# yuke93/ReconfigISP

Hardware: AMD Instinct MI355X
Metric: MPix/s end-to-end 5-stage ISP forward, 256x256 Bayer (higher is better)
Workload: dtype f32; 1 GPU; batch=64 256x256 Bayer per GPU, 5-stage fixed ISP forward Demosaic_01_sRGB_07_11_01_14 (nearest demosaic, bilateral denoise, WbManual, Gamma, GtmManual; OriginUniversal), all stage outputs materialised; global_batch=64, parallelism=batch-sharded x1, no collective

## Files before the change

reconfigisp_amd/csrc/risp_fused.hip:

```cpp
#include "risp_common.h"
#include "risp_ops.h"

namespace {

using namespace risp_ops;

constexpr int FX = 64, FY = 16, PXT = 4;

struct FusedArgs {
    const float *in;
    float *out_dem;
    float *out_bil;
    const int *win;
    const float *sig_c, *sig_s;
    int n_ops, N, H, W, R;
    int last_out;
    int ops[RISP_MAX_CHAIN];
    const float *params[RISP_MAX_CHAIN];
    float *outs[RISP_MAX_CHAIN];
};

__device__ __forceinline__ int refl(int i, int n) {
    if (i < 0) i = -i;
    if (i >= n) i = 2 * n - 2 - i;
    return i < 0 ? 0 : (i >= n ? n - 1 : i);
}
typedef float v4f __attribute__((ext_vector_type(4)));
__device__ __forceinline__ void st4_nt(float *p, v4f v) {
#ifndef RISP_STREAM_POLICY
#define RISP_STREAM_POLICY "nt"
#endif
    asm volatile("global_store_dwordx4 %0, %1, off " RISP_STREAM_POLICY ::"v"(p), "v"(v) : "memory");
}
__device__ __forceinline__ float q8f(float v) {
    return floorf(__builtin_amdgcn_fmed3f(v, 0.f, 255.f) + 0.5f);
}

template <bool FROM_BAYER, int RT, bool WBQ>
#ifndef RISP_FUSED_WAVES
#define RISP_FUSED_WAVES 1
#endif
__global__ __launch_bounds__(256, RISP_FUSED_WAVES) void bilateral_chain_kernel(const FusedArgs a) {
    extern __shared__ float lds[];
    const int R = RT > 0 ? RT : a.R, H = a.H, W = a.W;
    const int tw = FX + 2 * R, th = FY + 2 * R, per = tw * th;
#ifndef RISP_FUSED_NO_XCD_MAP
    int bxi = blockIdx.x, byi = blockIdx.y, bzi = blockIdx.z;
    {
        const unsigned total = gridDim.x * gridDim.y * gridDim.z;
        if ((total & 7u) == 0) {
            const unsigned lin = blockIdx.x + gridDim.x * (blockIdx.y + gridDim.y * blockIdx.z);
            const unsigned t = (lin & 7u) * (total >> 3) + (lin >> 3);
            bxi = t % gridDim.x;
            byi = (t / gridDim.x) % gridDim.y;
            bzi = t / (gridDim.x * gridDim.y);
        }
    }
    const int n = bzi, x0 = bxi * FX, y0 = byi * FY;
#else
    const int n = blockIdx.z, x0 = blockIdx.x * FX, y0 = blockIdx.y * FY;
#endif
    const size_t plane = (size_t)H * W;

    const int lx = (threadIdx.x & 15) * PXT, ly = threadIdx.x >> 4;
    const int px = x0 + lx, py = y0 + ly;
    if (FROM_BAYER && RT == 1) {
        constexpr int TWc = FX + 2, THc = FY + 2, PERc = TWc * THc, QW = FX / 2 + 2, QH = FY / 2 + 2;
        const float *bay = a.in + (size_t)n * plane;
        float2 top[2], bot[2];
#pragma unroll
        for (int it = 0; it < 2; ++it) {
            const int q = threadIdx.x + 256 * it;
            const int j = q / QW, i = q - j * QW;
            const int Y = y0 - 2 + 2 * j, X = x0 - 2 + 2 * i;
            const bool ok = q < QW * QH && Y >= 0 && Y < H && X >= 0 && X < W;
            top[it] = ok ? *reinterpret_cast<const float2 *>(bay + (size_t)Y * W + X) : make_float2(0.f, 0.f);
            bot[it] = ok ? *reinterpret_cast<const float2 *>(bay + (size_t)(Y + 1) * W + X) : make_float2(0.f, 0.f);
        }
#pragma unroll
        for (int it = 0; it < 2; ++it) {
            const int q = threadIdx.x + 256 * it;
            const int j = q / QW, i = q - j * QW;
            const int Y = y0 - 2 + 2 * j, X = x0 - 2 + 2 * i;
            if (!(q < QW * QH && Y >= 0 && Y < H && X >= 0 && X < W)) continue;
            const float R_ = top[it].x, G1 = top[it].y, G2 = bot[it].x, B_ = bot[it].y;
#pragma unroll
            for (int dy = 0; dy < 2; ++dy)
#pragma unroll
                for (int dx = 0; dx < 2; ++dx) {
                    const int ty = 2 * j - 1 + dy, tx = 2 * i - 1 + dx;
                    if (ty >= 0 && ty < THc && tx >= 0 && tx < TWc) {
                        const int idx = ty * TWc + tx;
                        lds[idx] = B_;
                        lds[PERc + idx] = dy ? G2 : G1;
                        lds[2 * PERc + idx] = R_;
                    }
                }
        }
        if (x0 == 0 || y0 == 0 || x0 + FX >= W || y0 + FY >= H) {
            __syncthreads();
            for (int idx = threadIdx.x; idx < PERc; idx += 256) {
                const int ty = idx / TWc, tx = idx - ty * TWc;
                const int gy = y0 - 1 + ty, gx = x0 - 1 + tx;
                if (gy >= 0 && gy < H && gx >= 0 && gx < W) continue;
                const int sy = refl(gy, H) - (y0 - 1), sx = refl(gx, W) - (x0 - 1);
                if (sy < 0 || sy >= THc || sx < 0 || sx >= TWc) continue;
                const int src = sy * TWc + sx;
                lds[idx] = lds[src];
                lds[PERc + idx] = lds[PERc + src];
                lds[2 * PERc + idx] = lds[2 * PERc + src];
            }
        }
    } else if (FROM_BAYER) {
        const float *bay = a.in + (size_t)n * plane;
        for (int idx = threadIdx.x; idx < per; idx += 256) {
            const int ty = idx / tw, tx = idx - ty * tw;
            const int gy = refl(y0 + ty - R, H), gx = refl(x0 + tx - R, W);
            const int qy = gy & ~1, qx = gx & ~1;
            lds[2 * per + idx] = bay[(size_t)qy * W + qx];
            lds[per + idx] = bay[(size_t)(qy + (gy & 1)) * W + qx + 1 - (gy & 1)];
            lds[idx] = bay[(size_t)(qy + 1) * W + qx + 1];
        }
    } else {
        const float *img = a.in + (size_t)n * 3 * plane;
        auto fetch1 = [&](int idx) {
            const int c = idx / per, rem = idx - c * per;
            const int ty = rem / tw, tx = rem - ty * tw;
            return img[(size_t)c * plane + (size_t)refl(y0 + ty - R, H) * W + refl(x0 + tx - R, W)];
        };
        if (RT > 0) {
            constexpr int PER3 = 3 * (FX + 2 * RT) * (FY + 2 * RT), NIT = (PER3 + 255) / 256;
            float v[NIT];
#pragma unroll
            for (int i = 0; i < NIT; ++i) {
                const int idx = threadIdx.x + 256 * i;
                v[i] = idx < PER3 ? fetch1(idx) : 0.f;
            }
#pragma unroll
            for (int i = 0; i < NIT; ++i) {
                const int idx = threadIdx.x + 256 * i;
                if (idx < PER3) lds[idx] = v[i];
            }
        } else {
            for (int idx = threadIdx.x; idx < 3 * per; idx += 256) lds[idx] = fetch1(idx);
        }
    }
    __syncthreads();

    if (px >= W || py >= H) return;
    const size_t o = (size_t)n * 3 * plane + (size_t)py * W + px;
    const float *ctr = lds + (ly + R) * tw + lx + R;

    if (FROM_BAYER) {
        float4 vb, vg, vr;
        float *eb = reinterpret_cast<float *>(&vb), *eg = reinterpret_cast<float *>(&vg), *er = reinterpret_cast<float *>(&vr);
#pragma unroll
        for (int i = 0; i < PXT; ++i) {
            eb[i] = ctr[i];
            eg[i] = ctr[per + i];
            er[i] = ctr[2 * per + i];
        }
        st4_nt(a.out_dem + o, *reinterpret_cast<v4f *>(&vb));
        st4_nt(a.out_dem + o + plane, *reinterpret_cast<v4f *>(&vg));
        st4_nt(a.out_dem + o + 2 * plane, *reinterpret_cast<v4f *>(&vr));
    }

    int r = a.win[n] / 2;
    r = r < 0 ? 0 : (r > R ? R : r);
    const bool full = RT > 0 && r == RT;
    const float ks = -1.f / (2.f * a.sig_s[n] * a.sig_s[n]), kc = -1.f / (2.f * a.sig_c[n] * a.sig_c[n]);
    const float ks2 = ks * 1.4426950408889634f, kc2 = kc * 1.4426950408889634f;
    f3 pix[PXT];
#pragma unroll
    for (int i = 0; i < PXT; ++i) {
        const float *c0 = ctr + i;
        const float cb = c0[0] * 255.f, cg = c0[per] * 255.f, cr = c0[2 * per] * 255.f;
        float nb = 0.f, ng = 0.f, nr = 0.f, den = 0.f;
        auto tap = [&](int dy, int dx) {
            if (dy == 0 && dx == 0) {
                nb += cb; ng += cg; nr += cr; den += 1.f;
                return;
            }
            const float *q = c0 + dy * tw + dx;
            const float qb = q[0] * 255.f, qg = q[per] * 255.f, qr = q[2 * per] * 255.f;
            const float dist = fabsf(qb - cb) + fabsf(qg - cg) + fabsf(qr - cr);
            const float wgt = __builtin_amdgcn_exp2f(__builtin_fmaf(dist * dist, kc2, (float)(dy * dy + dx * dx) * ks2));
            nb = __builtin_fmaf(wgt, qb, nb); ng = __builtin_fmaf(wgt, qg, ng); nr = __builtin_fmaf(wgt, qr, nr); den += wgt;
        };
        if (full) {
#pragma unroll
            for (int dy = -RT; dy <= RT; ++dy)
#pragma unroll
                for (int dx = -RT; dx <= RT; ++dx) tap(dy, dx);
        } else {
            for (int dy = -r; dy <= r; ++dy)
                for (int dx = -r; dx <= r; ++dx) tap(dy, dx);
        }
        const float inv255 = 1.f / 255.f, rden = 1.f / den;
        pix[i] = {q8f(nb * rden) * inv255, q8f(ng * rden) * inv255, q8f(nr * rden) * inv255};
    }
    auto store = [&](float *dst, bool stream) {
        const v4f vb = {pix[0].b, pix[1].b, pix[2].b, pix[3].b}, vg = {pix[0].g, pix[1].g, pix[2].g, pix[3].g},
                  vr = {pix[0].r, pix[1].r, pix[2].r, pix[3].r};
        if (stream) {
            st4_nt(dst + o, vb);
            st4_nt(dst + o + plane, vg);
            st4_nt(dst + o + 2 * plane, vr);
        } else {
            *reinterpret_cast<v4f *>(dst + o) = vb;
            *reinterpret_cast<v4f *>(dst + o + plane) = vg;
            *reinterpret_cast<v4f *>(dst + o + 2 * plane) = vr;
        }
    };
    store(a.out_bil, a.last_out >= 0);

    for (int k = 0; k < a.n_ops; ++k) {
        apply_op<PXT, WBQ>(a.ops[k], a.params[k], n, pix);
        if (a.outs[k]) store(a.outs[k], k < a.last_out);
    }
}

}

extern "C" {

int risp_bilateral_chain_fwd(const float *in, int from_bayer, float *out_demosaic, float *out_bilateral,
                             const int32_t *window, const float *sigma_color, const float *sigma_space, int max_window,
                             int n_ops, const int *ops, const float *const *params, float *const *outs, int N, int H,
                             int W, void *stream) {
    RISP_CHECK_ARG(in && out_bilateral && window && sigma_color && sigma_space, "risp_bilateral_chain_fwd: null argument");
    RISP_CHECK_ARG(!from_bayer || out_demosaic, "risp_bilateral_chain_fwd: demosaic output buffer missing");
    RISP_CHECK_ARG(n_ops >= 0 && n_ops <= RISP_MAX_CHAIN && (n_ops == 0 || (ops && params && outs)),
                   "risp_bilateral_chain_fwd: bad op list");
    RISP_CHECK_ARG(max_window >= 1 && max_window <= 17 && (max_window & 1), "risp_bilateral_chain_fwd: window %d", max_window);
    RISP_CHECK_ARG(N > 0 && N <= 65535 && H % 2 == 0 && W % 4 == 0 && H > max_window / 2 && W > max_window / 2,
                   "risp_bilateral_chain_fwd: bad shape N=%d H=%d W=%d (W must be a multiple of 4)", N, H, W);
    FusedArgs a;
    a.in = in;
    a.out_dem = out_demosaic;
    a.out_bil = out_bilateral;
    a.win = window;
    a.sig_c = sigma_color;
    a.sig_s = sigma_space;
    a.n_ops = n_ops;
    a.N = N;
    a.H = H;
    a.W = W;
    a.R = max_window / 2;
    a.last_out = -1;
    for (int k = 0; k < RISP_MAX_CHAIN; ++k) {
        a.ops[k] = RISP_OP_SKIP;
        a.params[k] = nullptr;
        a.outs[k] = nullptr;
    }
    for (int k = 0; k < n_ops; ++k) {
        RISP_CHECK_ARG(ops[k] == RISP_OP_SKIP || (ops[k] >= RISP_OP_WB_MANUAL && ops[k] <= RISP_OP_GAIN3),
                       "risp_bilateral_chain_fwd: op %d not allowed after the stencil", ops[k]);
        RISP_CHECK_ARG(ops[k] == RISP_OP_SKIP || (params[k] && outs[k]), "risp_bilateral_chain_fwd: stage %d incomplete", k);
        a.ops[k] = ops[k];
        a.params[k] = params[k];
        a.outs[k] = ops[k] == RISP_OP_SKIP ? nullptr : outs[k];
        if (a.outs[k]) a.last_out = k;
    }
#ifdef RISP_NT_ALL
    a.last_out = RISP_MAX_CHAIN;
#endif
    const size_t lds = sizeof(float) * 3 * (FX + 2 * a.R) * (FY + 2 * a.R);
    dim3 grid((W + FX - 1) / FX, (H + FY - 1) / FY, N);
    hipStream_t s = (hipStream_t)stream;
    bool wbq = false;
    for (int k = 0; k < n_ops; ++k) wbq |= a.ops[k] == RISP_OP_WB_QUADRATIC;
#ifdef RISP_CHAIN_ALWAYS_WBQ
    wbq = true;
#endif
#define RISP_FUSED_LAUNCH(FB, RTV)                                                                            \
    do {                                                                                                      \
        if (wbq) hipLaunchKernelGGL((bilateral_chain_kernel<FB, RTV, true>), grid, dim3(256), lds, s, a);     \
        else hipLaunchKernelGGL((bilateral_chain_kernel<FB, RTV, false>), grid, dim3(256), lds, s, a);        \
    } while (0)
    if (a.R == 1) {
        if (from_bayer) RISP_FUSED_LAUNCH(true, 1);
        else RISP_FUSED_LAUNCH(false, 1);
    } else {
        if (from_bayer) RISP_FUSED_LAUNCH(true, 0);
        else RISP_FUSED_LAUNCH(false, 0);
    }
#undef RISP_FUSED_LAUNCH
    RISP_LAUNCH_CHECK("risp_bilateral_chain_fwd");
    return 0;
}

const char *risp_bilateral_chain_kernel(int from_bayer, int max_window, int with_wb_quadratic) {
    static const char *names[2][2][2] = {
        {{"bilateral_chain_kernel<false,0,false>", "bilateral_chain_kernel<false,0,true>"},
         {"bilateral_chain_kernel<false,1,false>", "bilateral_chain_kernel<false,1,true>"}},
        {{"bilateral_chain_kernel<true,0,false>", "bilateral_chain_kernel<true,0,true>"},
         {"bilateral_chain_kernel<true,1,false>", "bilateral_chain_kernel<true,1,true>"}}};
    return names[from_bayer ? 1 : 0][max_window / 2 == 1 ? 1 : 0][with_wb_quadratic ? 1 : 0];
}

}
```

Before: 89660 MPix/s.

## Add register-only quad kernel for Bayer demosaic plus 3x3 bilateral chain

Adds a new kernel for the Bayer-input, radius-1 case. Each thread loads a 6x8 Bayer neighbourhood straight from global memory into registers, does the nearest demosaic and 3x3 bilateral filter on a 2x4 output patch, then runs the rest of the op chain, with no LDS and no barriers. The aim is to drop the shared-memory staging, the syncs and the tile halo overhead, in exchange for redundant global loads across neighbouring threads and more register pressure. The XCD remap is also moved into a helper, and the inline-asm nontemporal store gains an s_nop, while the new path uses the builtin nontemporal store.

```diff
diff --git a/reconfigisp_amd/csrc/risp_fused.hip b/reconfigisp_amd/csrc/risp_fused.hip
--- a/reconfigisp_amd/csrc/risp_fused.hip
+++ b/reconfigisp_amd/csrc/risp_fused.hip
@@ -30,10 +30,28 @@
 #ifndef RISP_STREAM_POLICY
 #define RISP_STREAM_POLICY "nt"
 #endif
-    asm volatile("global_store_dwordx4 %0, %1, off " RISP_STREAM_POLICY ::"v"(p), "v"(v) : "memory");
+    asm volatile("global_store_dwordx4 %0, %1, off " RISP_STREAM_POLICY "\n\ts_nop 1" ::"v"(p), "v"(v) : "memory");
+}
+__device__ __forceinline__ void st4_stream(float *p, v4f v) {
+    asm("" : "+v"(v));
+    __builtin_nontemporal_store(v, reinterpret_cast<v4f *>(p));
 }
 __device__ __forceinline__ float q8f(float v) {
     return floorf(__builtin_amdgcn_fmed3f(v, 0.f, 255.f) + 0.5f);
+}
+
+__device__ __forceinline__ void xcd_tile(int &bx, int &by, int &bz) {
+    bx = blockIdx.x, by = blockIdx.y, bz = blockIdx.z;
+#ifndef RISP_FUSED_NO_XCD_MAP
+    const unsigned total = gridDim.x * gridDim.y * gridDim.z;
+    if ((total & 7u) == 0) {
+        const unsigned lin = blockIdx.x + gridDim.x * (blockIdx.y + gridDim.y * blockIdx.z);
+        const unsigned t = (lin & 7u) * (total >> 3) + (lin >> 3);
+        bx = t % gridDim.x;
+        by = (t / gridDim.x) % gridDim.y;
+        bz = t / (gridDim.x * gridDim.y);
+    }
+#endif
 }
 
 template <bool FROM_BAYER, int RT, bool WBQ>
@@ -44,22 +62,9 @@
     extern __shared__ float lds[];
     const int R = RT > 0 ? RT : a.R, H = a.H, W = a.W;
     const int tw = FX + 2 * R, th = FY + 2 * R, per = tw * th;
-#ifndef RISP_FUSED_NO_XCD_MAP
-    int bxi = blockIdx.x, byi = blockIdx.y, bzi = blockIdx.z;
-    {
-        const unsigned total = gridDim.x * gridDim.y * gridDim.z;
-        if ((total & 7u) == 0) {
-            const unsigned lin = blockIdx.x + gridDim.x * (blockIdx.y + gridDim.y * blockIdx.z);
-            const unsigned t = (lin & 7u) * (total >> 3) + (lin >> 3);
-            bxi = t % gridDim.x;
-            byi = (t / gridDim.x) % gridDim.y;
-            bzi = t / (gridDim.x * gridDim.y);
-        }
-    }
+    int bxi, byi, bzi;
+    xcd_tile(bxi, byi, bzi);
     const int n = bzi, x0 = bxi * FX, y0 = byi * FY;
-#else
-    const int n = blockIdx.z, x0 = blockIdx.x * FX, y0 = blockIdx.y * FY;
-#endif
     const size_t plane = (size_t)H * W;
 
     const int lx = (threadIdx.x & 15) * PXT, ly = threadIdx.x >> 4;
@@ -220,6 +225,132 @@
     }
 }
 
+#ifndef RISP_QUAD_TX
+#define RISP_QUAD_TX 16
+#endif
+constexpr int QTX = RISP_QUAD_TX, QTY = 256 / QTX;
+static_assert(QTX * QTY == 256, "RISP_QUAD_TX must divide 256");
+
+template <bool WBQ>
+__global__ __launch_bounds__(256) void bilateral_chain_quad_kernel(const FusedArgs a) {
+    const int H = a.H, W = a.W;
+    int bxi, byi, bzi;
+    xcd_tile(bxi, byi, bzi);
+    const int n = bzi;
+    const int px = (bxi * QTX + (int)(threadIdx.x % QTX)) * 4, py = (byi * QTY + (int)(threadIdx.x / QTX)) * 2;
+    if (px >= W || py >= H) return;
+    const size_t plane = (size_t)H * W;
+
+    const float *bay = a.in + (size_t)n * plane;
+    const int j = py >> 1, i = px >> 1, qh = H >> 1, qw = W >> 1;
+    const int jr[3] = {j > 0 ? j - 1 : 0, j, j + 1 < qh ? j + 1 : qh - 1};
+    const int xl = 2 * (i > 0 ? i - 1 : 0), xr = 2 * (i + 2 < qw ? i + 2 : qw - 1);
+    float2 ml[6], mr[6];
+    float4 mc[6];
+#pragma unroll
+    for (int k = 0; k < 6; ++k) {
+        const float *row = bay + (size_t)(2 * jr[k >> 1] + (k & 1)) * W;
+        ml[k] = *reinterpret_cast<const float2 *>(row + xl);
+        mc[k] = *reinterpret_cast<const float4 *>(row + px);
+        mr[k] = *reinterpret_cast<const float2 *>(row + xr);
+    }
+    float qb[3][4], qg[3][4][2], qr[3][4];
+#pragma unroll
+    for (int k = 0; k < 3; ++k) {
+        const float2 e[4] = {ml[2 * k], make_float2(mc[2 * k].x, mc[2 * k].y), make_float2(mc[2 * k].z, mc[2 * k].w), mr[2 * k]};
+        const float2 o[4] = {ml[2 * k + 1], make_float2(mc[2 * k + 1].x, mc[2 * k + 1].y),
+                             make_float2(mc[2 * k + 1].z, mc[2 * k + 1].w), mr[2 * k + 1]};
+#pragma unroll
+        for (int c = 0; c < 4; ++c) {
+            qr[k][c] = e[c].x;
+            qg[k][c][0] = e[c].y;
+            qg[k][c][1] = o[c].x;
+            qb[k][c] = o[c].y;
+        }
+    }
+    const size_t o = (size_t)n * 3 * plane + (size_t)py * W + px;
+
+#pragma unroll
+    for (int p = 0; p < 2; ++p) {
+        const v4f vb = {qb[1][1], qb[1][1], qb[1][2], qb[1][2]}, vg = {qg[1][1][p], qg[1][1][p], qg[1][2][p], qg[1][2][p]},
+                  vr = {qr[1][1], qr[1][1], qr[1][2], qr[1][2]};
+        st4_stream(a.out_dem + o + (size_t)p * W, vb);
+        st4_stream(a.out_dem + o + (size_t)p * W + plane, vg);
+        st4_stream(a.out_dem + o + (size_t)p * W + 2 * plane, vr);
+    }
+
+#pragma unroll
+    for (int k = 0; k < 3; ++k)
+#pragma unroll
+        for (int c = 0; c < 4; ++c) {
+            qb[k][c] *= 255.f; qg[k][c][0] *= 255.f; qg[k][c][1] *= 255.f; qr[k][c] *= 255.f;
+        }
+    const bool full = a.win[n] / 2 >= 1;
+    const float ks = -1.f / (2.f * a.sig_s[n] * a.sig_s[n]), kc = -1.f / (2.f * a.sig_c[n] * a.sig_c[n]);
+    const float ks2 = ks * 1.4426950408889634f, kc2 = kc * 1.4426950408889634f;
+    f3 pix[2][PXT];
+#pragma unroll
+    for (int p = 0; p < 2; ++p)
+#pragma unroll
+        for (int c = 0; c < PXT; ++c) {
+            const float cb = qb[1][1 + c / 2], cg = qg[1][1 + c / 2][p], cr = qr[1][1 + c / 2];
+            float nb = 0.f, ng = 0.f, nr = 0.f, den = 0.f;
+            auto tap = [&](int dy, int dx) {
+                if (dy == 0 && dx == 0) {
+                    nb += cb; ng += cg; nr += cr; den += 1.f;
+                    return;
+                }
+                const int ty = 2 + p + dy, tx = 2 + c + dx;
+                const float tb = qb[ty / 2][tx / 2], tg = qg[ty / 2][tx / 2][ty & 1], tr = qr[ty / 2][tx / 2];
+                const float dist = fabsf(tb - cb) + fabsf(tg - cg) + fabsf(tr - cr);
+                const float wgt = __builtin_amdgcn_exp2f(__builtin_fmaf(dist * dist, kc2, (float)(dy * dy + dx * dx) * ks2));
+                nb = __builtin_fmaf(wgt, tb, nb); ng = __builtin_fmaf(wgt, tg, ng); nr = __builtin_fmaf(wgt, tr, nr); den += wgt;
+            };
+            if (full) {
+#pragma unroll
+                for (int dy = -1; dy <= 1; ++dy)
+#pragma unroll
+                    for (int dx = -1; dx <= 1; ++dx) tap(dy, dx);
+            } else {
+                tap(0, 0);
+            }
+            const float inv255 = 1.f / 255.f, rden = 1.f / den;
+            pix[p][c] = {q8f(nb * rden) * inv255, q8f(ng * rden) * inv255, q8f(nr * rden) * inv255};
+        }
+    auto store = [&](float *dst, bool stream) {
+#pragma unroll
+        for (int p = 0; p < 2; ++p) {
+            const v4f vb = {pix[p][0].b, pix[p][1].b, pix[p][2].b, pix[p][3].b}, vg = {pix[p][0].g, pix[p][1].g, pix[p][2].g, pix[p][3].g},
+                      vr = {pix[p][0].r, pix[p][1].r, pix[p][2].r, pix[p][3].r};
+            float *d = dst + o + (size_t)p * W;
+            if (stream) {
+                st4_stream(d, vb);
+                st4_stream(d + plane, vg);
+                st4_stream(d + 2 * plane, vr);
+            } else {
+                *reinterpret_cast<v4f *>(d) = vb;
+                *reinterpret_cast<v4f *>(d + plane) = vg;
+                *reinterpret_cast<v4f *>(d + 2 * plane) = vr;
+            }
+        }
+    };
+    store(a.out_bil, a.last_out >= 0);
+
+    for (int k = 0; k < a.n_ops; ++k) {
+        apply_op<2 * PXT, WBQ>(a.ops[k], a.params[k], n, &pix[0][0]);
+        if (a.outs[k]) store(a.outs[k], k < a.last_out);
+    }
+}
+
+}
+
+static bool quad_form(int from_bayer, int max_window) {
+#ifdef RISP_FUSED_LDS_FORM
+    (void)from_bayer, (void)max_window;
+    return false;
+#else
+    return from_bayer && max_window / 2 == 1;
+#endif
 }
 
 extern "C" {
@@ -278,7 +409,11 @@
         if (wbq) hipLaunchKernelGGL((bilateral_chain_kernel<FB, RTV, true>), grid, dim3(256), lds, s, a);     \
         else hipLaunchKernelGGL((bilateral_chain_kernel<FB, RTV, false>), grid, dim3(256), lds, s, a);        \
     } while (0)
-    if (a.R == 1) {
+    if (quad_form(from_bayer, max_window) && reinterpret_cast<uintptr_t>(in) % 16 == 0) {
+        const dim3 qgrid((W / 4 + QTX - 1) / QTX, (H / 2 + QTY - 1) / QTY, N);
+        if (wbq) hipLaunchKernelGGL((bilateral_chain_quad_kernel<true>), qgrid, dim3(256), 0, s, a);
+        else hipLaunchKernelGGL((bilateral_chain_quad_kernel<false>), qgrid, dim3(256), 0, s, a);
+    } else if (a.R == 1) {
         if (from_bayer) RISP_FUSED_LAUNCH(true, 1);
         else RISP_FUSED_LAUNCH(false, 1);
     } else {
@@ -291,6 +426,8 @@
 }
 
 const char *risp_bilateral_chain_kernel(int from_bayer, int max_window, int with_wb_quadratic) {
+    if (quad_form(from_bayer, max_window))
+        return with_wb_quadratic ? "bilateral_chain_quad_kernel<true>" : "bilateral_chain_quad_kernel<false>";
     static const char *names[2][2][2] = {
         {{"bilateral_chain_kernel<false,0,false>", "bilateral_chain_kernel<false,0,true>"},
          {"bilateral_chain_kernel<false,1,false>", "bilateral_chain_kernel<false,1,true>"}},
```

After: 96270 MPix/s (median of 6 runs). +7.4%, better.
